# AleoNet/snarkVM

Measured on NVIDIA H100. Metric: bls12_377_g1_msm_points_per_sec, higher is better.
Workload: dtype u32 limbs (Montgomery integer arithmetic, IMAD pipe)

## Files before the change

snarkvm_b200/csrc/cta_inverse.cuh:

```cuda
#pragma once
#include "ff.cuh"

namespace b200 {

static constexpr int CTA_INV_THREADS = 128;
static constexpr int CTA_INV_SMEM_BYTES = CTA_INV_THREADS * 48;
FF_DEV Fq shfl_up_fq(const Fq& a, int d) {
    Fq r;
#pragma unroll
    for (int j = 0; j < 12; j++) r.v[j] = __shfl_up_sync(0xffffffffu, a.v[j], d);
    return r;
}
FF_DEV Fq shfl_down_fq(const Fq& a, int d) {
    Fq r;
#pragma unroll
    for (int j = 0; j < 12; j++) r.v[j] = __shfl_down_sync(0xffffffffu, a.v[j], d);
    return r;
}
FF_DEV Fq shfl_idx_fq(const Fq& a, int l) {
    Fq r;
#pragma unroll
    for (int j = 0; j < 12; j++) r.v[j] = __shfl_sync(0xffffffffu, a.v[j], l);
    return r;
}
static __device__ __noinline__ Fq cta_shared_inverse(const Fq& run, uint32_t* sh) {
    const int tid = threadIdx.x, lane = tid & 31, warp = tid >> 5;
    run.store(sh + tid * 12);
    __syncthreads();
    if (warp == (int)(blockIdx.x & 3u)) {
        uint32_t* mine = sh + lane * 48;
        Fq a0 = Fq::load(mine), a1 = Fq::load(mine + 12), a2 = Fq::load(mine + 24), a3 = Fq::load(mine + 36);
        Fq p1 = a0 * a1, p2 = p1 * a2, p3 = p2 * a3;
        Fq incl = p3, suff = p3;
#pragma unroll 1
        for (int d = 1; d < 32; d <<= 1) {
            Fq up = shfl_up_fq(incl, d), dn = shfl_down_fq(suff, d);
            if (lane >= d) incl = incl * up;
            if (lane + d < 32) suff = suff * dn;
        }
        Fq tinv = shfl_idx_fq(incl, 31).inverse();
        Fq before = shfl_up_fq(incl, 1), after = shfl_down_fq(suff, 1);
        Fq ip3 = tinv;
        if (lane > 0) ip3 = ip3 * before;
        if (lane < 31) ip3 = ip3 * after;
        Fq ip2 = ip3 * a3, ip1 = ip2 * a2;
        (ip3 * p2).store(mine + 36);
        (ip2 * p1).store(mine + 24);
        (ip1 * a0).store(mine + 12);
        (ip1 * a1).store(mine);
    }
    __syncthreads();
    return Fq::load(sh + tid * 12);
}

static __device__ __noinline__ Fq cta_shared_inverse_by(const Fq& run, uint32_t* sh, int inv_warp) {
    const int tid = threadIdx.x, lane = tid & 31, warp = tid >> 5;
    run.store(sh + tid * 12);
    __syncthreads();
    if (warp == inv_warp) {
        uint32_t* mine = sh + lane * 48;
        Fq a0 = Fq::load(mine), a1 = Fq::load(mine + 12), a2 = Fq::load(mine + 24), a3 = Fq::load(mine + 36);
        Fq p1 = a0 * a1, p2 = p1 * a2, p3 = p2 * a3;
        Fq incl = p3, suff = p3;
#pragma unroll 1
        for (int d = 1; d < 32; d <<= 1) {
            Fq up = shfl_up_fq(incl, d), dn = shfl_down_fq(suff, d);
            if (lane >= d) incl = incl * up;
            if (lane + d < 32) suff = suff * dn;
        }
        Fq tinv = coop_inverse<FqParams>(shfl_idx_fq(incl, 31));
        Fq before = shfl_up_fq(incl, 1), after = shfl_down_fq(suff, 1);
        Fq ip3 = tinv;
        if (lane > 0) ip3 = ip3 * before;
        if (lane < 31) ip3 = ip3 * after;
        Fq ip2 = ip3 * a3, ip1 = ip2 * a2;
        (ip3 * p2).store(mine + 36);
        (ip2 * p1).store(mine + 24);
        (ip1 * a0).store(mine + 12);
        (ip1 * a1).store(mine);
    }
    __syncthreads();
    return Fq::load(sh + tid * 12);
}


}
```

snarkvm_b200/csrc/ff.cuh:

```cuda
#pragma once
#include <cstdint>
#include <cuda_runtime.h>

namespace b200 {

#define FF_DEV __device__ __forceinline__

FF_DEV uint32_t ptx_add_cc(uint32_t a, uint32_t b) { uint32_t r; asm volatile("add.cc.u32 %0, %1, %2;" : "=r"(r) : "r"(a), "r"(b)); return r; }
FF_DEV uint32_t ptx_addc_cc(uint32_t a, uint32_t b) { uint32_t r; asm volatile("addc.cc.u32 %0, %1, %2;" : "=r"(r) : "r"(a), "r"(b)); return r; }
FF_DEV uint32_t ptx_addc(uint32_t a, uint32_t b) { uint32_t r; asm volatile("addc.u32 %0, %1, %2;" : "=r"(r) : "r"(a), "r"(b)); return r; }
FF_DEV uint32_t ptx_sub_cc(uint32_t a, uint32_t b) { uint32_t r; asm volatile("sub.cc.u32 %0, %1, %2;" : "=r"(r) : "r"(a), "r"(b)); return r; }
FF_DEV uint32_t ptx_subc_cc(uint32_t a, uint32_t b) { uint32_t r; asm volatile("subc.cc.u32 %0, %1, %2;" : "=r"(r) : "r"(a), "r"(b)); return r; }
FF_DEV uint32_t ptx_subc(uint32_t a, uint32_t b) { uint32_t r; asm volatile("subc.u32 %0, %1, %2;" : "=r"(r) : "r"(a), "r"(b)); return r; }
FF_DEV uint32_t ptx_mul_lo(uint32_t a, uint32_t b) { uint32_t r; asm volatile("mul.lo.u32 %0, %1, %2;" : "=r"(r) : "r"(a), "r"(b)); return r; }
FF_DEV uint32_t ptx_mul_hi(uint32_t a, uint32_t b) { uint32_t r; asm volatile("mul.hi.u32 %0, %1, %2;" : "=r"(r) : "r"(a), "r"(b)); return r; }
FF_DEV uint32_t ptx_mad_lo_cc(uint32_t a, uint32_t b, uint32_t c) { uint32_t r; asm volatile("mad.lo.cc.u32 %0, %1, %2, %3;" : "=r"(r) : "r"(a), "r"(b), "r"(c)); return r; }
FF_DEV uint32_t ptx_madc_lo_cc(uint32_t a, uint32_t b, uint32_t c) { uint32_t r; asm volatile("madc.lo.cc.u32 %0, %1, %2, %3;" : "=r"(r) : "r"(a), "r"(b), "r"(c)); return r; }
FF_DEV uint32_t ptx_madc_hi_cc(uint32_t a, uint32_t b, uint32_t c) { uint32_t r; asm volatile("madc.hi.cc.u32 %0, %1, %2, %3;" : "=r"(r) : "r"(a), "r"(b), "r"(c)); return r; }
FF_DEV uint32_t ptx_madc_hi(uint32_t a, uint32_t b, uint32_t c) { uint32_t r; asm volatile("madc.hi.u32 %0, %1, %2, %3;" : "=r"(r) : "r"(a), "r"(b), "r"(c)); return r; }

FF_DEV uint32_t ptx_neg(uint32_t x) { uint32_t r; asm volatile("sub.u32 %0, 0, %1;" : "=r"(r) : "r"(x)); return r; }

template <int N>
FF_DEV void row_mul(uint32_t (&acc)[N], const uint32_t* x, uint32_t y) {
// ... 339 lines not shown
        return pow_const<N>(e);
    }

    FF_DEV Fp half() const {
        uint32_t t[N + 1];
        if (v[0] & 1u) {
            t[0] = ptx_add_cc(v[0], P::mod(0));
#pragma unroll
            for (int i = 1; i < N; i++) t[i] = ptx_addc_cc(v[i], P::mod(i));
            t[N] = ptx_addc(0u, 0u);
        } else {
#pragma unroll
            for (int i = 0; i < N; i++) t[i] = v[i];
            t[N] = 0u;
        }
        Fp r;
#pragma unroll
        for (int i = 0; i < N; i++) r.v[i] = __funnelshift_r(t[i], t[i + 1], 1);
        return r;
    }

    FF_DEV Fp to_mont() const { return (*this) * r2(); }
    FF_DEV Fp from_mont() const { Fp o = zero(); o.v[0] = 1u; return (*this) * o; }

    FF_DEV static Fp load(const void* p) {
        Fp r; const uint4* q = reinterpret_cast<const uint4*>(p);
#pragma unroll
        for (int i = 0; i < N / 4; i++) { uint4 t = q[i]; r.v[4 * i] = t.x; r.v[4 * i + 1] = t.y; r.v[4 * i + 2] = t.z; r.v[4 * i + 3] = t.w; }
        return r;
    }
    FF_DEV static Fp load_ldg(const void* p) {
        Fp r; const uint4* q = reinterpret_cast<const uint4*>(p);
#pragma unroll
        for (int i = 0; i < N / 4; i++) { uint4 t = __ldg(q + i); r.v[4 * i] = t.x; r.v[4 * i + 1] = t.y; r.v[4 * i + 2] = t.z; r.v[4 * i + 3] = t.w; }
        return r;
    }
    FF_DEV void store(void* p) const {
        uint4* q = reinterpret_cast<uint4*>(p);
#pragma unroll
        for (int i = 0; i < N / 4; i++) q[i] = make_uint4(v[4 * i], v[4 * i + 1], v[4 * i + 2], v[4 * i + 3]);
    }
};

FF_DEV uint32_t coop_carries_in(uint32_t gen, uint32_t prop) {
    const uint32_t a = gen | prop;
    return (a + gen) ^ a ^ gen;
}
template <class P>
FF_DEV uint32_t coop_mod_limb(int lane) {
    uint32_t p = 0u;
#pragma unroll
    for (int k = 0; k < P::N; k++) if (lane == k) p = P::mod(k);
    return p;
}
template <class P>
FF_DEV uint32_t coop_mul(uint32_t a, uint32_t b, uint32_t p, int lane) {
    constexpr int N = P::N;
    uint32_t lo = 0u, hi = 0u, ex = 0u;
    uint32_t bi = __shfl_sync(0xffffffffu, b, 0);
#pragma unroll
    for (int i = 0; i < N; i++) {
        const uint32_t bnext = __shfl_sync(0xffffffffu, b, (i + 1) % N);
        asm("mad.lo.cc.u32 %0, %3, %4, %0; madc.hi.cc.u32 %1, %3, %4, %1; addc.u32 %2, %2, 0;" : "+r"(lo), "+r"(hi), "+r"(ex) : "r"(a), "r"(bi));
        const uint32_t m = __shfl_sync(0xffffffffu, lo * P::INV32, 0);
        asm("mad.lo.cc.u32 %0, %3, %4, %0; madc.hi.cc.u32 %1, %3, %4, %1; addc.u32 %2, %2, 0;" : "+r"(lo), "+r"(hi), "+r"(ex) : "r"(m), "r"(p));
        const uint32_t t = __shfl_down_sync(0xffffffffu, lo, 1);
        asm("add.cc.u32 %0, %1, %3; addc.u32 %1, %2, 0;" : "=r"(lo), "+r"(hi), "+r"(ex) : "r"(t));
        ex = 0u;
        bi = bnext;
    }
    uint32_t up = __shfl_up_sync(0xffffffffu, hi, 1);
    if (lane == 0) up = 0u;
    uint32_t s = lo + up;
    const uint32_t cin = coop_carries_in(__ballot_sync(0xffffffffu, s < up), __ballot_sync(0xffffffffu, s == 0xffffffffu));
    s += (cin >> lane) & 1u;
    const uint32_t gt = __ballot_sync(0xffffffffu, s > p), lt = __ballot_sync(0xffffffffu, s < p);
    if (gt >= lt) {
        const uint32_t bin = coop_carries_in(lt, __ballot_sync(0xffffffffu, s == p));
        s = s - p - ((bin >> lane) & 1u);
    }
    return s;
}
template <class P>
FF_DEV Fp<P> coop_inverse(const Fp<P>& v) {
    constexpr int N = P::N;
    const int lane = threadIdx.x & 31;
    const uint32_t p = coop_mod_limb<P>(lane);
    uint32_t x = 0u;
#pragma unroll
    for (int k = 0; k < N; k++) if (lane == k) x = v.v[k];
    uint32_t acc = x;
    bool started = false;
#pragma unroll 1
    for (int i = N - 1; i >= 0; i--) {
        uint32_t e = 0u, borrow_in = 0u;
#pragma unroll
        for (int k = 0; k < N; k++) {
            const uint32_t mk = P::mod(k), sub = (k == 0 ? 2u : 0u) + borrow_in;
            const uint32_t ek = mk - sub;
            borrow_in = (mk < sub) ? 1u : 0u;
            if (k == i) e = ek;
        }
#pragma unroll 1
        for (int b = 31; b >= 0; b--) {
            if (started) acc = coop_mul<P>(acc, acc, p, lane);
            if ((e >> b) & 1u) { acc = started ? coop_mul<P>(acc, x, p, lane) : x; started = true; }
        }
    }
    Fp<P> r;
#pragma unroll
    for (int k = 0; k < N; k++) r.v[k] = __shfl_sync(0xffffffffu, acc, k);
    return r;
}

#define FF_TABLE(name, ...) \
    __host__ __device__ static constexpr uint32_t name(int i) { constexpr uint32_t t[N] = {__VA_ARGS__}; return t[i]; }

struct FrParams {
    static constexpr int N = 8;
    static constexpr uint32_t INV32 = 0xffffffffu;
    static constexpr bool MOD0_IS_ONE = true;
    FF_TABLE(mod, 0x00000001u, 0x0a118000u, 0xd0000001u, 0x59aa76feu, 0x5c37b001u, 0x60b44d1eu, 0x9a2ca556u, 0x12ab655eu)
    FF_TABLE(r1,  0xfffffff3u, 0x7d1c7fffu, 0x6ffffff2u, 0x7257f50fu, 0x512c0feeu, 0x16d81575u, 0x2bbb9a9du, 0x0d4bda32u)
    FF_TABLE(r2,  0xb861857bu, 0x25d577bau, 0x8860591fu, 0xcc2c27b5u, 0xe5dc8593u, 0xa7cc008fu, 0xeff1c939u, 0x011fdae7u)
};
struct FqParams {
    static constexpr int N = 12;
    static constexpr uint32_t INV32 = 0xffffffffu;
    static constexpr bool MOD0_IS_ONE = true;
    FF_TABLE(mod, 0x00000001u, 0x8508c000u, 0x30000000u, 0x170b5d44u, 0xba094800u, 0x1ef3622fu, 0x00f5138fu, 0x1a22d9f3u, 0x6ca1493bu, 0xc63b05c0u, 0x17c510eau, 0x01ae3a46u)
    FF_TABLE(r1,  0xffffff68u, 0x02cdffffu, 0x7fffffb1u, 0x51409f83u, 0x8a7d3ff2u, 0x9f7db3a9u, 0x6e7c6305u, 0x7b4e97b7u, 0x803c84e8u, 0x4cf495bfu, 0xe2fdf49au, 0x008d6661u)
    FF_TABLE(r2,  0x9400cd22u, 0xb786686cu, 0xb00431b1u, 0x0329fcaau, 0x62d6b46du, 0x22a5f111u, 0x827dc3acu, 0xbfdf7d03u, 0x41790bf9u, 0x837e92f0u, 0x1e914b88u, 0x006dfccbu)
};
#undef FF_TABLE

using Fr = Fp<FrParams>;
using Fq = Fp<FqParams>;

}
```

snarkvm_b200/csrc/msm.cu:

```cuda
#include "msm.cuh"

#include <atomic>
#include <condition_variable>
#include <memory>
#include <mutex>
#include <utility>
#include <vector>
#include <cstdio>
#include <cstdlib>
#include <cstring>
#include <cub/device/device_scan.cuh>

#define FF_CALL_MUL 1
#include "ec.cuh"
#include "cta_inverse.cuh"
#include "quad.cuh"
#define FIELD_TEST_ENTRY test_field_op_msm
#include "testops.cuh"

namespace b200 {

static std::atomic<uint64_t> g_launches{0};
uint64_t launch_count() { return g_launches.load(); }
void count_launch(int n) { g_launches.fetch_add((uint64_t)n); }
// ... 376 lines not shown
                                                        uint32_t* __restrict__ dense_out) {
    __shared__ uint4 sh_inv4[PAIR_THREADS * 3];
    uint32_t* sh_inv = reinterpret_cast<uint32_t*>(sh_inv4);
    const uint32_t total = off_out[total_buckets];
    const uint64_t o0_64 = (uint64_t)(blockIdx.x * blockDim.x + threadIdx.x) * T;
    const uint32_t o0 = o0_64 < total ? (uint32_t)o0_64 : total;
    const uint32_t o1 = (o0_64 + T < total) ? o0 + T : total;
    uint32_t lo = 0, hi = total_buckets;
    if (o0 < o1) while (hi - lo > 1) { uint32_t mid = (lo + hi) >> 1; if (off_out[mid] <= o0) lo = mid; else hi = mid; }
    uint32_t b = lo;

    Fq run = Fq::one();
    for (uint32_t o = o0; o < o1; o++) {
        while (o >= off_out[b + 1]) b++;
        const uint32_t i = o - off_out[b], base_in = off_in[b], cnt = off_in[b + 1] - base_in;
        const bool has2 = 2 * i + 1 < cnt;
        if (has2) {
            const uint32_t* pp = level_input_ptr<GATHER>(dense_bases, sorted, dense_in, base_in + 2 * i);
            const uint32_t* qp = level_input_ptr<GATHER>(dense_bases, sorted, dense_in, base_in + 2 * i + 1);
            Fq x1 = Fq::load_ldg(pp), x2 = Fq::load_ldg(qp);
            if (x1 == x2 || x1.is_zero() || x2.is_zero()) {
                DensePoint P = load_level_input<GATHER>(dense_bases, sorted, dense_in, base_in + 2 * i);
                DensePoint Q = load_level_input<GATHER>(dense_bases, sorted, dense_in, base_in + 2 * i + 1);
                Fq d;
                int kind = classify_pair(P, Q, true, d);
                if (kind >= PAIR_ADD) run = run * d;
            } else {
                run = run * (x2 - x1);
            }
        }
        run.store(prefix + (size_t)o * 12);
    }
    Fq inv = cta_shared_inverse(run, sh_inv);
    for (uint32_t o = o1; o-- > o0;) {
        while (o < off_out[b]) b--;
        const uint32_t i = o - off_out[b], base_in = off_in[b], cnt = off_in[b + 1] - base_in;
        const bool has2 = 2 * i + 1 < cnt;
        DensePoint P = load_level_input<GATHER>(dense_bases, sorted, dense_in, base_in + 2 * i);
        DensePoint Q = P;
        if (has2) Q = load_level_input<GATHER>(dense_bases, sorted, dense_in, base_in + 2 * i + 1);
        Fq d;
        int kind = classify_pair(P, Q, has2, d);
        DensePoint R;
        if (kind == PAIR_COPY1) R = P;
        else if (kind == PAIR_COPY2) R = Q;
        else if (kind == PAIR_INF) { R.inf = true; R.x = Fq::zero(); R.y = Fq::zero(); }
        else {
            Fq inv_d = (o == o0) ? inv : inv * Fq::load(prefix + (size_t)(o - 1) * 12);
            inv = inv * d;
            Fq lambda;
            if (kind == PAIR_ADD) lambda = (Q.y - P.y) * inv_d;
            else { Fq xx = P.x.sqr(); lambda = (xx.dbl() + xx) * inv_d; }
            Fq x3 = lambda.sqr() - P.x - Q.x;
            R.y = lambda * (P.x - x3) - P.y;
            R.x = x3;
            R.inf = false;
        }
        store_dense(dense_out + (size_t)o * DENSE_WORDS, R);
    }
}


FF_DEV uint32_t smem_addr_u32(const void* p) { return (uint32_t)__cvta_generic_to_shared(p); }
FF_DEV void cp_async16(uint32_t dst, const void* src) {
    asm volatile("cp.async.cg.shared.global [%0], [%1], 16;" ::"r"(dst), "l"(src) : "memory");
}
FF_DEV void cp_async_commit() { asm volatile("cp.async.commit_group;" ::: "memory"); }
FF_DEV void cp_async_wait_1() { asm volatile("cp.async.wait_group 1;" ::: "memory"); }
FF_DEV void cp_async_wait_0() { asm volatile("cp.async.wait_group 0;" ::: "memory"); }
FF_DEV void cp_async_wait_3() { asm volatile("cp.async.wait_group 3;" ::: "memory"); }

static constexpr int RING_CHUNKS = 12;
static constexpr int RING_STAGE_U4 = RING_CHUNKS * 32;
static constexpr int PAIR2_SMEM = PAIR_THREADS * 48 + 4 * 2 * RING_STAGE_U4 * 16;

FF_DEV Fq ring_fq(const uint4* slot) {
    Fq r;
#pragma unroll
    for (int i = 0; i < 3; i++) { uint4 t = slot[i * 32]; r.v[4 * i] = t.x; r.v[4 * i + 1] = t.y; r.v[4 * i + 2] = t.z; r.v[4 * i + 3] = t.w; }
    return r;
}

static constexpr uint32_t PAIR_NONE = 0xffffffffu;
template <bool GATHER>
__global__ void __launch_bounds__(256) k_pair_desc(const uint32_t* __restrict__ sorted, const uint32_t* __restrict__ off_in,
                                                   const uint32_t* __restrict__ off_out, uint32_t total_buckets, uint2* __restrict__ desc,
                                                   const uint32_t* __restrict__ in_base_ptr ) {
    const uint32_t o = blockIdx.x * blockDim.x + threadIdx.x;
    if (o >= __ldg(off_out + total_buckets)) return;
    uint32_t lo = 0, hi = total_buckets;
    while (hi - lo > 1) { uint32_t mid = (lo + hi) >> 1; if (__ldg(off_out + mid) <= o) lo = mid; else hi = mid; }
    const uint32_t i = o - __ldg(off_out + lo), base_in = __ldg(off_in + lo), cnt = __ldg(off_in + lo + 1) - base_in;
    const uint32_t idx = base_in + 2u * i;
    const bool has2 = 2u * i + 1u < cnt;
    uint2 d;
    if (GATHER) { d.x = __ldg(sorted + idx); d.y = has2 ? __ldg(sorted + idx + 1) : PAIR_NONE; }
    else { d.x = idx - (in_base_ptr ? __ldg(in_base_ptr) : 0u); d.y = has2 ? 0u : PAIR_NONE; }
    desc[o] = d;
}

struct PairDesc {
    uint32_t p, q;
    bool valid;
    FF_DEV bool has2() const { return valid && q != PAIR_NONE; }
};
FF_DEV PairDesc pair_load_desc(int64_t j, uint32_t nv, const uint2* __restrict__ dlane) {
    PairDesc d; d.p = 0; d.q = PAIR_NONE; d.valid = false;
    if (j < 0 || j >= (int64_t)nv) return d;
    const uint2 v = __ldg(dlane + 32 * j);
    d.p = v.x; d.q = v.y; d.valid = true;
    return d;
}
template <bool GATHER>
FF_DEV const uint32_t* pair_src(const PairDesc& d, int which, const uint32_t* __restrict__ records) {
    if (GATHER) return records + (size_t)((which ? d.q : d.p) & 0x7fffffffu) * BASE_WORDS;
    return records + (size_t)(d.p + (uint32_t)which) * DENSE_WORDS;
}
template <bool GATHER, bool FULL>
FF_DEV void pair_issue(const PairDesc& d, uint4* ring, int st, int lane, const uint32_t* __restrict__ records, int chunks) {
    if (d.valid) {
        const uint32_t dst = smem_addr_u32(ring + (size_t)st * (size_t)(chunks * 32) + lane);
        const uint32_t* p = pair_src<GATHER>(d, 0, records);
#pragma unroll
        for (int k = 0; k < (FULL ? 6 : 3); k++) cp_async16(dst + (uint32_t)k * 512u, p + 4 * k);
        if (d.q != PAIR_NONE) {
            const uint32_t* q = pair_src<GATHER>(d, 1, records);
#pragma unroll
            for (int k = 0; k < (FULL ? 6 : 3); k++) cp_async16(dst + (uint32_t)((FULL ? 6 : 3) + k) * 512u, q + 4 * k);
        }
    }
    cp_async_commit();
}
template <bool GATHER>
FF_DEV int pair_classify_global(const PairDesc& d, const uint32_t* __restrict__ records, Fq& den) {
    DensePoint P = load_dense(pair_src<GATHER>(d, 0, records));
    DensePoint Q = load_dense(pair_src<GATHER>(d, 1, records));
    if (GATHER) { if ((d.p >> 31) && !P.inf) P.y = P.y.neg(); if ((d.q >> 31) && !Q.inf) Q.y = Q.y.neg(); }
    return classify_pair(P, Q, true, den);
}

template <bool GATHER, int MINB>
__global__ void __launch_bounds__(PAIR_THREADS, MINB) k_pair_level2(const uint32_t* __restrict__ records ,
                                                         const uint2* __restrict__ desc, const uint32_t* __restrict__ total_ptr,
                                                         uint32_t T_bound, uint32_t* __restrict__ prefix, uint32_t* __restrict__ dense_out,
                                                         uint32_t* __restrict__ sm_slots) {
    (void)T_bound;
    extern __shared__ uint4 pair2_smem[];
    __shared__ uint32_t sh_slot;
    uint32_t* sh_inv = reinterpret_cast<uint32_t*>(pair2_smem);
    const int lane = threadIdx.x & 31, warp = threadIdx.x >> 5;
    uint4* ring = pair2_smem + PAIR_THREADS * 3 + (size_t)warp * 2 * RING_STAGE_U4;
    if (threadIdx.x == 0) {
        uint32_t smid;
        asm volatile("mov.u32 %0, %%smid;" : "=r"(smid));
        sh_slot = atomicAdd(sm_slots + (smid & 255u), 1u);
    }
    __syncthreads();
    const int inv_warp = (int)(sh_slot & 3u);
    const uint32_t total = __ldg(total_ptr);
    const uint64_t lanes = (uint64_t)gridDim.x * PAIR_THREADS;
    const uint32_t T = total > lanes ? (uint32_t)((total + lanes - 1) / lanes) : 1u;
    const uint64_t w0_64 = ((uint64_t)blockIdx.x * (PAIR_THREADS / 32) + (uint32_t)warp) * 32ull * T + (uint32_t)lane;
    uint32_t nv = 0;
    if (w0_64 < total) { const uint64_t left = (total - w0_64 + 31) / 32; nv = left < T ? (uint32_t)left : T; }
    const uint2* dlane = desc + w0_64;
    uint32_t* plane = prefix + w0_64 * 12;
    uint32_t* olane = dense_out + w0_64 * DENSE_WORDS;

    Fq run = Fq::one();
    {
        constexpr int PF = 3;
        PairDesc q0 = pair_load_desc(0, nv, dlane), q1 = pair_load_desc(1, nv, dlane), q2 = pair_load_desc(2, nv, dlane);
        pair_issue<GATHER, false>(q0, ring, 0, lane, records, 6);
        pair_issue<GATHER, false>(q1, ring, 1, lane, records, 6);
        pair_issue<GATHER, false>(q2, ring, 2, lane, records, 6);
        PairDesc ahead = pair_load_desc(PF, nv, dlane);
        for (uint32_t j = 0; j < T; j++) {
            pair_issue<GATHER, false>(ahead, ring, (int)((j + PF) & 3u), lane, records, 6);
            const PairDesc cur = q0;
            q0 = q1; q1 = q2; q2 = ahead;
            ahead = pair_load_desc((int64_t)j + PF + 1, nv, dlane);
// ... 874 lines not shown
            const uint32_t w0 = set_of(u0), wn = set_of(u0 + un) - w0;
            const uint32_t tb = wn * plan.nbuckets;
            const uint32_t* bs = bucket_start + (size_t)w0 * plan.nbuckets;
            const SetOffsets so = set_offsets(plan, flat, w0);
            size_t entries = set_cap * (size_t)un;
            if (entries > max_entries) entries = max_entries;
            if (large_hot) CUDA_TRY(cudaMemsetAsync(hot_dev, 0, 4, stream));
            size_t items_bound = 1;
            size_t items_launched = 1;
            const uint32_t* final_partial = nullptr;
            const uint32_t* final_start = nullptr;
            if (levels == 0) {
                const uint32_t cap = (acc_g8 || acc_q8 || small_cap) ? item_cap : plan.cap;
                k_items_per_bucket<<<(tb + 256) / 256, 256, 0, stream>>>(hist + (size_t)w0 * plan.nbuckets, items, tb, cap, (quad_fold || large_hot) ? hot_dev : nullptr, (uint32_t)hot_max, hot_keep);
                CUDA_TRY(cub::DeviceScan::ExclusiveSum(cub_tmp, cub_bytes, items, item_start, (int)(tb + 1), stream));
                count_launch(2);
                const size_t group_items = (size_t)tb + entries / cap + 1;
                items_bound = set_cap / cap + 1;
                items_launched = group_items;
                ProfScope acc_scope(PROF_MSM_ACCUMULATE, stream);
                if (acc_q8) {
                    k_bucket_accumulate_q8<<<(unsigned)((group_items * 32 + 127) / 128), 128, 0, stream>>>(gather_src, sorted, bs, item_start, tb, cap, partial);
                    items_bound = 1;
                } else if (acc_g8)
                    k_bucket_accumulate_g8<<<(unsigned)((group_items * ACC_G + 127) / 128), 128, 0, stream>>>(gather_src, sorted, bs, item_start, tb, cap, partial);
                else
                    k_bucket_accumulate<<<(unsigned)((group_items + MSM_ACC_THREADS - 1) / MSM_ACC_THREADS), MSM_ACC_THREADS, 0, stream>>>(
                        gather_src, sorted, bs, item_start, tb, cap, partial);
                count_launch();
            } else {
                if (records) {
                    ProfScope sort_scope(PROF_MSM_SORT, stream);
                    for (int i = 0; i < nsegs; i++) {
                        const MsmSegment& sg = segs[i];
                        if (sg.n == 0) continue;
                        const int64_t first = (int64_t)sg.job * wins_per_job;
                        int w_lo, w_hi;
                        if (flat) {
                            if (first < (int64_t)u0 || first >= (int64_t)u0 + un) continue;
                            w_lo = 0; w_hi = plan.nwin;
                        } else {
                            const int64_t lo_w = (int64_t)u0 - first, hi_w = (int64_t)u0 + un - first;
                            w_lo = lo_w < 0 ? 0 : (int)lo_w; w_hi = hi_w > plan.nwin ? plan.nwin : (int)hi_w;
                            if (w_lo >= w_hi) continue;
                        }
                        const unsigned grid = (unsigned)((sg.n + 255) / 256);
                        const uint32_t slot_base = sg.job * sets_per_job * plan.nbuckets;
                        const uint32_t* sc = (const uint32_t*)sg.d_scalars;
                        const int ct = plan.c_top, nw = plan.nwin;
                        if (flat) {
                            if (sg.mont) k_scatter_records<true, true><<<grid, 256, 0, stream>>>(sc, sg.n, nullptr, 0, table, table_n, plan.c, ct, nw, plan.nbuckets, cursors, slot_base, w_lo, w_hi, bs, (uint4*)dense0);
                            else k_scatter_records<false, true><<<grid, 256, 0, stream>>>(sc, sg.n, nullptr, 0, table, table_n, plan.c, ct, nw, plan.nbuckets, cursors, slot_base, w_lo, w_hi, bs, (uint4*)dense0);
                        } else {
                            if (sg.mont) k_scatter_records<true, false><<<grid, 256, 0, stream>>>(sc, sg.n, seg_points[i], seg_stride[i], nullptr, 0, plan.c, ct, nw, plan.nbuckets, cursors, slot_base, w_lo, w_hi, bs, (uint4*)dense0);
                            else k_scatter_records<false, false><<<grid, 256, 0, stream>>>(sc, sg.n, seg_points[i], seg_stride[i], nullptr, 0, plan.c, ct, nw, plan.nbuckets, cursors, slot_base, w_lo, w_hi, bs, (uint4*)dense0);
                        }
                        count_launch();
                    }
                }
                ProfScope acc_scope(PROF_MSM_ACCUMULATE, stream);
                const uint32_t* off_in = bs;
                uint32_t* off_bufs[2] = {off_a, off_b};
                uint32_t* dense_bufs[2] = {dense_a, dense_b};
                const uint32_t* dense_in = records ? dense0 : nullptr;
                size_t bound = entries;
                for (int l = 0; l < levels; l++) {
                    uint32_t* off_out = off_bufs[l & 1];
                    uint32_t* dense_out = dense_bufs[l & 1];
                    k_halve_counts<<<(tb + 256) / 256, 256, 0, stream>>>(off_in, cnt_tmp, tb);
                    CUDA_TRY(cub::DeviceScan::ExclusiveSum(cub_tmp, cub_bytes, cnt_tmp, off_out, (int)(tb + 1), stream));
                    bound = bound / 2 + tb;
                    const size_t wave = (size_t)sm_count * (pair_v1 ? 4 : pair_minb) * 128;
                    size_t waves = (bound + 1024 * wave - 1) / (1024 * wave);
                    if (pair_waves) waves = pair_waves;
                    size_t T = (bound + waves * wave - 1) / (waves * wave);
                    const size_t nthreads = (bound + T - 1) / T;
                    const unsigned lgrid = (unsigned)((nthreads + 127) / 128);
                    if (pair_v1) {
                        if (l == 0 && !records)
                            k_pair_level<true><<<lgrid, 128, 0, stream>>>(gather_src, sorted, nullptr, off_in, off_out, tb, (uint32_t)T, prefix, dense_out);
                        else
                            k_pair_level<false><<<lgrid, 128, 0, stream>>>(nullptr, nullptr, dense_in, off_in, off_out, tb, (uint32_t)T, prefix, dense_out);
                    } else {
                        const unsigned dgrid = (unsigned)((bound + 255) / 256);
                        if (l == 0 && !records) {
                            k_pair_desc<true><<<dgrid, 256, 0, stream>>>(sorted, off_in, off_out, tb, desc, nullptr);
                            if (pair_minb == 3) k_pair_level2<true, 3><<<lgrid, 128, PAIR2_SMEM, stream>>>(gather_src, desc, off_out + tb, (uint32_t)T, prefix, dense_out, sm_slots);
                            else k_pair_level2<true, 4><<<lgrid, 128, PAIR2_SMEM, stream>>>(gather_src, desc, off_out + tb, (uint32_t)T, prefix, dense_out, sm_slots);
                        } else {
                            k_pair_desc<false><<<dgrid, 256, 0, stream>>>(nullptr, off_in, off_out, tb, desc, l == 0 ? bs : nullptr);
                            if (pair_minb == 3) k_pair_level2<false, 3><<<lgrid, 128, PAIR2_SMEM, stream>>>(dense_in, desc, off_out + tb, (uint32_t)T, prefix, dense_out, sm_slots);
                            else k_pair_level2<false, 4><<<lgrid, 128, PAIR2_SMEM, stream>>>(dense_in, desc, off_out + tb, (uint32_t)T, prefix, dense_out, sm_slots);
                        }
                        count_launch(1);
                    }
                    count_launch(3);
                    off_in = off_out;
                    dense_in = dense_out;
                }
                k_items_from_offsets<<<(tb + 256) / 256, 256, 0, stream>>>(off_in, items, tb, plan.cap, large_hot ? hot_dev : nullptr, (uint32_t)hot_max, hot_keep);
                CUDA_TRY(cub::DeviceScan::ExclusiveSum(cub_tmp, cub_bytes, items, item_start, (int)(tb + 1), stream));
                const size_t group_items = (size_t)tb + bound / plan.cap + 1;
                items_bound = ((set_cap >> levels) + 1) / plan.cap + 1;
                items_launched = group_items;
                k_bucket_accumulate_dense<<<(unsigned)((group_items + MSM_ACC_THREADS - 1) / MSM_ACC_THREADS), MSM_ACC_THREADS, 0, stream>>>(
                    dense_in, off_in, item_start, tb, plan.cap, partial);
                count_launch(3);
            }
            ProfScope red_scope(PROF_MSM_REDUCE, stream);
            int quad_rounds = 0;
            if (quad_fold) {
                size_t worst = acc_q8 ? 1 : items_bound;
                const uint32_t* p_in = partial; uint32_t* p_out = partial2;
                while (worst > 32) {
                    k_fold_hot_quad<<<(unsigned)sm_count * 8, 128, 0, stream>>>(p_in, item_start, hot_dev, (uint32_t)hot_max, (uint32_t)quad_rounds, 32u, p_out);
                    count_launch();
                    worst = (worst + 31) / 32;
                    quad_rounds++;
                    const uint32_t* t1 = p_in; p_in = p_out; p_out = (uint32_t*)t1;
                }
                final_partial = partial; final_start = item_start;
            } else if (large_hot) {
                size_t worst = items_bound;
                const uint32_t* p_in = partial; uint32_t* p_out = partial2;
                while (worst > 1) {
                    k_fold_hot_quad<<<(unsigned)sm_count * 8, 128, 0, stream>>>(p_in, item_start, hot_dev, (uint32_t)hot_max, (uint32_t)quad_rounds, 1u, p_out);
                    count_launch();
                    worst = (worst + 31) / 32;
                    quad_rounds++;
                    const uint32_t* t1 = p_in; p_in = p_out; p_out = (uint32_t*)t1;
                }
                final_partial = partial; final_start = item_start;
            } else {
                size_t worst = items_bound;
                size_t total_bound = items_launched;
                uint32_t* p_in = partial; uint32_t* p_out = partial2;
                uint32_t* st_in = item_start; uint32_t* st_out = items2;
                while (worst > 1) {
                    k_group_counts<<<(tb + 256) / 256, 256, 0, stream>>>(st_in, cnt_tmp, tb);
                    CUDA_TRY(cub::DeviceScan::ExclusiveSum(cub_tmp, cub_bytes, cnt_tmp, st_out, (int)(tb + 1), stream));
                    const size_t out_bound = (size_t)tb + total_bound / 32 + 1;
                    total_bound = out_bound;
                    k_partial_group_sum<<<(unsigned)((out_bound + 127) / 128), 128, 0, stream>>>(p_in, st_in, st_out, tb, p_out);
                    count_launch(3);
                    worst = (worst + 31) / 32;
                    uint32_t* t1 = p_in; p_in = p_out; p_out = t1;
                    uint32_t* t2 = st_in; st_in = st_out; st_out = t2;
                }
                final_partial = p_in; final_start = st_in;
            }
            uint32_t* group_sums = d_window_sums + (size_t)w0 * XYZZ_WORDS;
            if (warp_reduce && quad_path != 0) {
                const uint32_t qchunks = (plan.nbuckets + 7u) / 8u;
                k_bucket_reduce_quad<<<(wn * qchunks * 32u + 127u) / 128u, 128, 0, stream>>>(final_partial, quad_fold ? partial2 : final_partial, final_start,
                                                                                              quad_rounds, plan.nbuckets, qchunks, wn, red_a);
                const uint32_t* ent = red_a;
                uint32_t m = qchunks;
                int lgw = 3;
                if (m > 64u) {
                    const uint32_t groups = (m + 7u) / 8u;
                    k_combine_level_quad<<<(wn * groups * 32u + 127u) / 128u, 128, 0, stream>>>(ent, m, wn, lgw, red_b);
                    count_launch();
                    ent = red_b; m = groups; lgw += 3;
                }
                k_window_combine_quad<<<wn, 32u * ((m + 7u) / 8u), 0, stream>>>(ent, m, lgw, group_sums, so);
                count_launch(2);
                continue;
            }
            if (warp_reduce) {
                const uint32_t wchunks = (plan.nbuckets + 31u) / 32u;
                k_bucket_reduce_warp<<<(wn * wchunks * 32u + 127u) / 128u, 128, 0, stream>>>(final_partial, final_start, plan.nbuckets, wchunks, wn, red_a);
                k_window_combine_warp<<<wn, 32, 0, stream>>>(red_a, wchunks, group_sums, so);
                count_launch(2);
// ... 379 lines not shown
```

Baseline: 158.6 million.

## Use safegcd divstep inversion and merge-path tiled pair descriptors

Replaces the warp-cooperative Fermat exponentiation inverse with a per-thread Bernstein-Yang safegcd (30-bit limb divsteps) inverse, aiming to remove the long chain of cooperative modular multiplications. The CTA batch-inverse code is restructured to shorten register live ranges by reloading inputs after the scan. k_pair_desc is rewritten to use merge-path splitting with tiles of bucket offsets staged in shared memory, replacing a per-output global binary search. The new inverse carries a correctness risk in its constant-time bound and final normalisation, and the descriptor kernel adds per-block split searches.

New measurement: 165.2 million, median of 6. 1.04x the previous value.

```diff
diff --git a/snarkvm_b200/csrc/cta_inverse.cuh b/snarkvm_b200/csrc/cta_inverse.cuh
--- a/snarkvm_b200/csrc/cta_inverse.cuh
+++ b/snarkvm_b200/csrc/cta_inverse.cuh
@@ -59,20 +59,24 @@
     __syncthreads();
     if (warp == inv_warp) {
         uint32_t* mine = sh + lane * 48;
-        Fq a0 = Fq::load(mine), a1 = Fq::load(mine + 12), a2 = Fq::load(mine + 24), a3 = Fq::load(mine + 36);
-        Fq p1 = a0 * a1, p2 = p1 * a2, p3 = p2 * a3;
-        Fq incl = p3, suff = p3;
+        Fq total, others;
+        {
+            const Fq a0 = Fq::load(mine), a1 = Fq::load(mine + 12), a2 = Fq::load(mine + 24), a3 = Fq::load(mine + 36);
+            const Fq p3 = a0 * a1 * a2 * a3;
+            Fq incl = p3, suff = p3;
 #pragma unroll 1
-        for (int d = 1; d < 32; d <<= 1) {
-            Fq up = shfl_up_fq(incl, d), dn = shfl_down_fq(suff, d);
-            if (lane >= d) incl = incl * up;
-            if (lane + d < 32) suff = suff * dn;
+            for (int d = 1; d < 32; d <<= 1) {
+                Fq up = shfl_up_fq(incl, d), dn = shfl_down_fq(suff, d);
+                if (lane >= d) incl = incl * up;
+                if (lane + d < 32) suff = suff * dn;
+            }
+            total = shfl_idx_fq(incl, 31);
+            const Fq before = shfl_up_fq(incl, 1), after = shfl_down_fq(suff, 1);
+            others = lane == 0 ? after : lane == 31 ? before : before * after;
         }
-        Fq tinv = coop_inverse<FqParams>(shfl_idx_fq(incl, 31));
-        Fq before = shfl_up_fq(incl, 1), after = shfl_down_fq(suff, 1);
-        Fq ip3 = tinv;
-        if (lane > 0) ip3 = ip3 * before;
-        if (lane < 31) ip3 = ip3 * after;
+        const Fq ip3 = coop_inverse<FqParams>(total) * others;
+        const Fq a0 = Fq::load(mine), a1 = Fq::load(mine + 12), a2 = Fq::load(mine + 24), a3 = Fq::load(mine + 36);
+        const Fq p1 = a0 * a1, p2 = p1 * a2;
         Fq ip2 = ip3 * a3, ip1 = ip2 * a2;
         (ip3 * p2).store(mine + 36);
         (ip2 * p1).store(mine + 24);
diff --git a/snarkvm_b200/csrc/ff.cuh b/snarkvm_b200/csrc/ff.cuh
--- a/snarkvm_b200/csrc/ff.cuh
+++ b/snarkvm_b200/csrc/ff.cuh
@@ -445,35 +445,95 @@
     return s;
 }
 template <class P>
+__host__ __device__ constexpr int mod_bits() {
+    int b = 32 * (P::N - 1);
+    for (uint32_t t = P::mod(P::N - 1); t; t >>= 1) b++;
+    return b;
+}
+template <class P>
+__host__ __device__ constexpr int32_t const_limb30(bool r2, int i) {
+    const int w = 30 * i / 32, s = 30 * i % 32;
+    const uint64_t lo = w < P::N ? (r2 ? P::r2(w) : P::mod(w)) : 0u, hi = w + 1 < P::N ? (r2 ? P::r2(w + 1) : P::mod(w + 1)) : 0u;
+    return (int32_t)(((lo | hi << 32) >> s) & 0x3fffffffu);
+}
+template <class P>
+__host__ __device__ constexpr uint32_t mod_inv30() {
+    uint32_t x = P::mod(0);
+    for (int i = 0; i < 5; i++) x *= 2u - P::mod(0) * x;
+    return x & 0x3fffffffu;
+}
+
+template <class P>
 FF_DEV Fp<P> coop_inverse(const Fp<P>& v) {
-    constexpr int N = P::N;
-    const int lane = threadIdx.x & 31;
-    const uint32_t p = coop_mod_limb<P>(lane);
-    uint32_t x = 0u;
-#pragma unroll
-    for (int k = 0; k < N; k++) if (lane == k) x = v.v[k];
-    uint32_t acc = x;
-    bool started = false;
+    constexpr int N = P::N, L = (mod_bits<P>() + 2 + 29) / 30, BATCHES = ((49 * mod_bits<P>() + 57) / 17 + 29) / 30;
+    constexpr int32_t M30 = 0x3fffffff;
+    constexpr uint32_t PINV = mod_inv30<P>();
+    static_assert(mod_bits<P>() >= 46 && (P::mod(0) & 1u), "the divstep bound and the odd modulus");
+    int32_t f[L], g[L], d[L], e[L];
+#pragma unroll
+    for (int i = 0; i < L; i++) {
+        const int w = 30 * i / 32, s = 30 * i % 32;
+        const uint64_t lo = w < N ? v.v[w] : 0u, hi = w + 1 < N ? v.v[w + 1] : 0u;
+        g[i] = (int32_t)(((lo | hi << 32) >> s) & (uint64_t)M30);
+        f[i] = const_limb30<P>(false, i);
+        d[i] = 0;
+        e[i] = const_limb30<P>(true, i);
+    }
+    int32_t delta = 1;
 #pragma unroll 1
-    for (int i = N - 1; i >= 0; i--) {
-        uint32_t e = 0u, borrow_in = 0u;
-#pragma unroll
-        for (int k = 0; k < N; k++) {
-            const uint32_t mk = P::mod(k), sub = (k == 0 ? 2u : 0u) + borrow_in;
-            const uint32_t ek = mk - sub;
-            borrow_in = (mk < sub) ? 1u : 0u;
-            if (k == i) e = ek;
-        }
-#pragma unroll 1
-        for (int b = 31; b >= 0; b--) {
-            if (started) acc = coop_mul<P>(acc, acc, p, lane);
-            if ((e >> b) & 1u) { acc = started ? coop_mul<P>(acc, x, p, lane) : x; started = true; }
-        }
-    }
-    Fp<P> r;
-#pragma unroll
-    for (int k = 0; k < N; k++) r.v[k] = __shfl_sync(0xffffffffu, acc, k);
-    return r;
+    for (int it = 0; it < BATCHES; it++) {
+        uint32_t fl = (uint32_t)f[0], gl = (uint32_t)g[0];
+        int32_t u = 1, w = 0, q = 0, r = 1;
+#pragma unroll
+        for (int k = 0; k < 30; k++) {
+            const bool odd = gl & 1u, swap = odd && delta > 0;
+            if (swap) { delta = 1 - delta; const uint32_t t = gl; gl = (gl - fl) >> 1; fl = t; const int32_t tu = u, tw = w; u = 2 * q; w = 2 * r; q -= tu; r -= tw; }
+            else { delta = 1 + delta; if (odd) { gl = (gl + fl) >> 1; q += u; r += w; } else gl >>= 1; u *= 2; w *= 2; }
+        }
+        int64_t cf = (int64_t)u * f[0] + (int64_t)w * g[0], cg = (int64_t)q * f[0] + (int64_t)r * g[0];
+        cf >>= 30; cg >>= 30;
+#pragma unroll
+        for (int i = 1; i < L; i++) {
+            cf += (int64_t)u * f[i] + (int64_t)w * g[i];
+            cg += (int64_t)q * f[i] + (int64_t)r * g[i];
+            f[i - 1] = (int32_t)cf & M30; cf >>= 30;
+            g[i - 1] = (int32_t)cg & M30; cg >>= 30;
+        }
+        f[L - 1] = (int32_t)cf; g[L - 1] = (int32_t)cg;
+        const int32_t sd = d[L - 1] >> 31, se = e[L - 1] >> 31;
+        int32_t md = (u & sd) + (w & se), me = (q & sd) + (r & se);
+        int64_t cd = (int64_t)u * d[0] + (int64_t)w * e[0], ce = (int64_t)q * d[0] + (int64_t)r * e[0];
+        md -= (int32_t)((PINV * (uint32_t)cd + (uint32_t)md) & (uint32_t)M30);
+        me -= (int32_t)((PINV * (uint32_t)ce + (uint32_t)me) & (uint32_t)M30);
+        cd += (int64_t)const_limb30<P>(false, 0) * md; ce += (int64_t)const_limb30<P>(false, 0) * me;
+        cd >>= 30; ce >>= 30;
+#pragma unroll
+        for (int i = 1; i < L; i++) {
+            cd += (int64_t)u * d[i] + (int64_t)w * e[i] + (int64_t)const_limb30<P>(false, i) * md;
+            ce += (int64_t)q * d[i] + (int64_t)r * e[i] + (int64_t)const_limb30<P>(false, i) * me;
+            d[i - 1] = (int32_t)cd & M30; cd >>= 30;
+            e[i - 1] = (int32_t)ce & M30; ce >>= 30;
+        }
+        d[L - 1] = (int32_t)cd; e[L - 1] = (int32_t)ce;
+    }
+    const int32_t sd = d[L - 1] >> 31, sf = f[L - 1] >> 31;
+#pragma unroll
+    for (int i = 0; i < L; i++) d[i] = ((d[i] + (const_limb30<P>(false, i) & sd)) ^ sf) - sf;
+#pragma unroll
+    for (int i = 0; i < L - 1; i++) { d[i + 1] += d[i] >> 30; d[i] &= M30; }
+    const int32_t sn = d[L - 1] >> 31;
+#pragma unroll
+    for (int i = 0; i < L; i++) d[i] += const_limb30<P>(false, i) & sn;
+#pragma unroll
+    for (int i = 0; i < L - 1; i++) { d[i + 1] += d[i] >> 30; d[i] &= M30; }
+    Fp<P> res;
+#pragma unroll
+    for (int k = 0; k < N; k++) {
+        const int i = 32 * k / 30, s = 32 * k % 30;
+        const uint64_t x = (uint64_t)(uint32_t)d[i] >> s | (i + 1 < L ? (uint64_t)(uint32_t)d[i + 1] << (30 - s) : 0u);
+        res.v[k] = (uint32_t)x;
+    }
+    return res;
 }
 
 #define FF_TABLE(name, ...) \
diff --git a/snarkvm_b200/csrc/msm.cu b/snarkvm_b200/csrc/msm.cu
--- a/snarkvm_b200/csrc/msm.cu
+++ b/snarkvm_b200/csrc/msm.cu
@@ -482,21 +482,54 @@
 }
 
 static constexpr uint32_t PAIR_NONE = 0xffffffffu;
+static constexpr int DESC_THREADS = 256;
+static constexpr uint32_t DESC_TILE = 2048;
+
+FF_DEV uint32_t pair_desc_split(const uint32_t* __restrict__ off_out, uint32_t tb, uint32_t total, uint32_t d, int lane) {
+    uint32_t lo = d > total ? d - total : 0u, hi = d < tb ? d : tb;
+    while (lo < hi) {
+        const uint32_t step = (hi - lo + 31u) / 32u, i = lo + (uint32_t)lane * step;
+        const bool before = i < hi && __ldg(off_out + i + 1) <= d - 1u - i;
+        const uint32_t n = __popc(__ballot_sync(0xffffffffu, before));
+        if (n == 0) hi = lo;
+        else { const uint32_t top = lo + n * step; lo += (n - 1u) * step + 1u; if (top < hi) hi = top; }
+    }
+    return lo;
+}
+
 template <bool GATHER>
-__global__ void __launch_bounds__(256) k_pair_desc(const uint32_t* __restrict__ sorted, const uint32_t* __restrict__ off_in,
+__global__ void __launch_bounds__(DESC_THREADS) k_pair_desc(const uint32_t* __restrict__ sorted, const uint32_t* __restrict__ off_in,
                                                    const uint32_t* __restrict__ off_out, uint32_t total_buckets, uint2* __restrict__ desc,
                                                    const uint32_t* __restrict__ in_base_ptr ) {
-    const uint32_t o = blockIdx.x * blockDim.x + threadIdx.x;
-    if (o >= __ldg(off_out + total_buckets)) return;
-    uint32_t lo = 0, hi = total_buckets;
-    while (hi - lo > 1) { uint32_t mid = (lo + hi) >> 1; if (__ldg(off_out + mid) <= o) lo = mid; else hi = mid; }
-    const uint32_t i = o - __ldg(off_out + lo), base_in = __ldg(off_in + lo), cnt = __ldg(off_in + lo + 1) - base_in;
-    const uint32_t idx = base_in + 2u * i;
-    const bool has2 = 2u * i + 1u < cnt;
-    uint2 d;
-    if (GATHER) { d.x = __ldg(sorted + idx); d.y = has2 ? __ldg(sorted + idx + 1) : PAIR_NONE; }
-    else { d.x = idx - (in_base_ptr ? __ldg(in_base_ptr) : 0u); d.y = has2 ? 0u : PAIR_NONE; }
-    desc[o] = d;
+    __shared__ uint32_t sh_out[DESC_TILE + 1], sh_in[DESC_TILE + 2], sh_split[2];
+    const uint32_t tb = total_buckets, total = __ldg(off_out + tb);
+    const uint64_t items = (uint64_t)tb + total, d0_64 = (uint64_t)blockIdx.x * DESC_TILE;
+    if (d0_64 >= items) return;
+    const uint32_t d0 = (uint32_t)d0_64, d1 = (uint32_t)(items - d0_64 < DESC_TILE ? items : d0_64 + DESC_TILE);
+    if (threadIdx.x < 64) {
+        const uint32_t s = pair_desc_split(off_out, tb, total, threadIdx.x < 32 ? d0 : d1, (int)(threadIdx.x & 31));
+        if ((threadIdx.x & 31) == 0) sh_split[threadIdx.x >> 5] = s;
+    }
+    __syncthreads();
+    const uint32_t i0 = sh_split[0], i1 = sh_split[1], j0 = d0 - i0, j1 = d1 - i1, nb = i1 - i0;
+    for (uint32_t k = threadIdx.x; k <= nb + 1u; k += DESC_THREADS) {
+        if (i0 + k > tb) break;
+        if (k <= nb) sh_out[k] = __ldg(off_out + i0 + k);
+        sh_in[k] = __ldg(off_in + i0 + k);
+    }
+    __syncthreads();
+    const uint32_t in_base = GATHER || !in_base_ptr ? 0u : __ldg(in_base_ptr);
+    for (uint32_t o = j0 + threadIdx.x; o < j1; o += DESC_THREADS) {
+        uint32_t lo = 0, hi = nb + 1u;
+        while (hi - lo > 1u) { const uint32_t mid = (lo + hi) >> 1; if (sh_out[mid] <= o) lo = mid; else hi = mid; }
+        const uint32_t i = o - sh_out[lo], base_in = sh_in[lo], cnt = sh_in[lo + 1] - base_in;
+        const uint32_t idx = base_in + 2u * i;
+        const bool has2 = 2u * i + 1u < cnt;
+        uint2 d;
+        if (GATHER) { d.x = __ldg(sorted + idx); d.y = has2 ? __ldg(sorted + idx + 1) : PAIR_NONE; }
+        else { d.x = idx - in_base; d.y = has2 ? 0u : PAIR_NONE; }
+        desc[o] = d;
+    }
 }
 
 struct PairDesc {
@@ -1537,13 +1570,13 @@
                         else
                             k_pair_level<false><<<lgrid, 128, 0, stream>>>(nullptr, nullptr, dense_in, off_in, off_out, tb, (uint32_t)T, prefix, dense_out);
                     } else {
-                        const unsigned dgrid = (unsigned)((bound + 255) / 256);
+                        const unsigned dgrid = (unsigned)((bound + tb + DESC_TILE - 1) / DESC_TILE);
                         if (l == 0 && !records) {
-                            k_pair_desc<true><<<dgrid, 256, 0, stream>>>(sorted, off_in, off_out, tb, desc, nullptr);
+                            k_pair_desc<true><<<dgrid, DESC_THREADS, 0, stream>>>(sorted, off_in, off_out, tb, desc, nullptr);
                             if (pair_minb == 3) k_pair_level2<true, 3><<<lgrid, 128, PAIR2_SMEM, stream>>>(gather_src, desc, off_out + tb, (uint32_t)T, prefix, dense_out, sm_slots);
                             else k_pair_level2<true, 4><<<lgrid, 128, PAIR2_SMEM, stream>>>(gather_src, desc, off_out + tb, (uint32_t)T, prefix, dense_out, sm_slots);
                         } else {
-                            k_pair_desc<false><<<dgrid, 256, 0, stream>>>(nullptr, off_in, off_out, tb, desc, l == 0 ? bs : nullptr);
+                            k_pair_desc<false><<<dgrid, DESC_THREADS, 0, stream>>>(nullptr, off_in, off_out, tb, desc, l == 0 ? bs : nullptr);
                             if (pair_minb == 3) k_pair_level2<false, 3><<<lgrid, 128, PAIR2_SMEM, stream>>>(dense_in, desc, off_out + tb, (uint32_t)T, prefix, dense_out, sm_slots);
                             else k_pair_level2<false, 4><<<lgrid, 128, PAIR2_SMEM, stream>>>(dense_in, desc, off_out + tb, (uint32_t)T, prefix, dense_out, sm_slots);
                         }
```
